# cfpark00/vdm4cdm

Hardware: NVIDIA B200
Metric: denoiser voxel-steps/s at 128^3 (reverse ancestral sampling) (higher is better)
Workload: dtype bf16

## Files before the change

vdm4cdm_b200/csrc/conv3d.cu:

```cuda
#include "common.cuh"
#include "ptx.cuh"
#include "tma_host.cuh"

#ifdef VDM_BRINGUP
#define VDM_DBG(p, f) (((p).debug_flags & (f)) != 0)
#else
#define VDM_DBG(p, f) (false)
#endif

namespace vdm {

constexpr int kConvThreads = 512;
constexpr int kEpiThreads = 256;
constexpr int kEpiFirst = 128;
constexpr int kXfThreads = 128;
constexpr int kXfFirst = 384;
constexpr int kRegsWg0 = 64, kRegsEpi = 176, kRegsXf = 88;
constexpr int kXfGroup = 2;
constexpr int kResSlotBytes = 2 * 16 * kEpiThreads;
constexpr int kMaxBStages = 16;
constexpr int kMaxAStages = 4;
constexpr int kTileH = 16, kTileW = 8;

struct ConvKernelParams {
// ... 918 lines not shown
                issue_fold_stage<MT, KJ, NF>(a_st + kh * (uint32_t)(kTileW + 2) + kw, b_base16 + sb * b_stage16 + b_lbo, a_hi32,
                                             b_hi32, d_tmem0, kc == 0 && khw == 0);
                ptx::umma_commit(&sh->b_empty[sb]);
              }
              ptx::umma_commit(&sh->a_empty[sa]);
              if (kc == k_chunks - 1) ptx::umma_commit(&sh->tmem_full[acc]);
            }
            __syncwarp();
          }
        }
      } else {
      Ring ra(nsa_u);
      for (int tile = blockIdx.x; tile < p.n_tiles; tile += gridDim.x, ++ti) {
        const uint32_t acc = ti & 1;
        ptx::mbar_wait(&sh->tmem_empty[acc], ((ti >> 1) & 1) ^ 1);
        if (ti == 0) ptx::mbar_wait(&sh->b_full[0], 0);
        const uint32_t d_tmem0 = tmem_u + acc * (uint32_t)(MT * NF);
        const int total_chunks = k_chunks + p.skip_chunks;
        for (int kc = 0; kc < total_chunks; ++kc, ra.next()) {
          const uint32_t sa = ra.s;
          ptx::mbar_wait(&a_rdy[sa], ra.ph);
          ptx::tc_fence_after();
          if (leader) {
            if (kc == 0)
              issue_fold_tile<MT, KJ, NF, true>(a_base16 + sa * a_stage16, b_base16, a_hi, b_hi, d_tmem0);
            else if (kc < k_chunks)
              issue_fold_tile<MT, KJ, NF, false>(a_base16 + sa * a_stage16, b_base16 + (uint32_t)kc * chunk_b16, a_hi, b_hi,
                                                 d_tmem0);
            else
              issue_skip_chunk<MT, KJ, NF>(a_base16 + sa * a_stage16,
                                           b_base16 + ((uint32_t)p.b_stage_bytes >> 4) + (uint32_t)(kc - k_chunks) * (2u * KJ * NF),
                                           d_tmem0);
            ptx::umma_commit(&sh->a_empty[sa]);
            if (kc == total_chunks - 1) ptx::umma_commit(&sh->tmem_full[acc]);
          }
          __syncwarp();
        }
      }
      }
    } else {
      const bool res = p.b_resident != 0;
      if (!p.pad) {
        if (res) issue_generic_tiles<MT, KJ, 0, 1, true, kKind>(p, sh, a_rdy, a_base16, b_base16, tmem_u, leader);
        else issue_generic_tiles<MT, KJ, 0, 1, false, kKind>(p, sh, a_rdy, a_base16, b_base16, tmem_u, leader);
      } else if (p.taps_per_stage == 3) {
        if (res) issue_generic_tiles<MT, KJ, 1, 3, true, kKind>(p, sh, a_rdy, a_base16, b_base16, tmem_u, leader);
        else issue_generic_tiles<MT, KJ, 1, 3, false, kKind>(p, sh, a_rdy, a_base16, b_base16, tmem_u, leader);
      } else {
        if (res) issue_generic_tiles<MT, KJ, 1, 1, true, kKind>(p, sh, a_rdy, a_base16, b_base16, tmem_u, leader);
        else issue_generic_tiles<MT, KJ, 1, 1, false, kKind>(p, sh, a_rdy, a_base16, b_base16, tmem_u, leader);
      }
    }
  }
  } else if (warp >= 12) {
    ptx::setmaxnreg_dec<kRegsXf>();
    if constexpr (!TF32)
      if (p.in_norm) transform_tiles<MT, KJ>(p, sh, a_smem, reinterpret_cast<float*>(smem + p.xf_coef_off));
  } else {
    ptx::setmaxnreg_inc<kRegsEpi>();
    constexpr int P = TF32 ? kEpiF32Planar : 0;
    if (p.out_fp32) epilogue_tiles<MT, kEpiFp32>(p, sh, smem, stat_part, stat_acc, tmem_base);
    else if (p.residual && p.stats) epilogue_tiles<MT, P | kEpiRes | kEpiStats>(p, sh, smem, stat_part, stat_acc, tmem_base);
    else if (p.residual) epilogue_tiles<MT, P | kEpiRes>(p, sh, smem, stat_part, stat_acc, tmem_base);
    else if (p.stats) epilogue_tiles<MT, P | kEpiStats>(p, sh, smem, stat_part, stat_acc, tmem_base);
    else epilogue_tiles<MT, P>(p, sh, smem, stat_part, stat_acc, tmem_base);
  }

  ptx::tc_fence_before();
  __syncthreads();
  if (warp == 1) {
    ptx::tc_fence_after();
    ptx::tmem_dealloc(tmem_base, (uint32_t)p.tmem_cols);
  }
}

#include "conv3d_march.cuh"

struct ConvOverrides {
  int debug_flags;
  int force_mt, force_kc, force_nsplit;
  int no_resident;
  int no_fold;
  int no_march;
};
#ifdef VDM_BRINGUP
static ConvOverrides g_overrides = {};
#else
constexpr ConvOverrides g_overrides = {};
#endif

enum class ConvSchedule {
  kTile,
  kFoldResident,
  kFoldStreamed,
  kMarch,
};

struct ConvPlan {
  ConvSchedule schedule;
  int pad;
  int mt, kc, n_split, n_cta;
  int n_tiles, grid;
  int nsa, nsb, taps_per_stage;
  int a_stage_bytes, b_stage_bytes, b_resident;
  int res_depth, res_ring_off;
  int xf_coef_off;
  size_t smem_bytes;
  int m_units, m_nseg, m_seglen;
  int debug_flags;
};

static int tap_cell(const VdmConvDesc& d, int t) {
  return (d.tap_offset[t][0] + 1) * 9 + (d.tap_offset[t][1] + 1) * 3 + d.tap_offset[t][2] + 1;
}

static int plan_conv(const VdmConvDesc& d, bool has_residual, bool has_skip, bool has_xf, int skip_c_in, int sms, bool tf32,
                     ConvPlan& pl) {
  const ConvOverrides& ov = g_overrides;
  pl = ConvPlan{};
  pl.debug_flags = ov.debug_flags;
  int pad = 0;
  for (int t = 0; t < d.n_taps; ++t)
    if (d.tap_offset[t][0] != 0 || d.tap_offset[t][1] != 0 || d.tap_offset[t][2] != 0) pad = 1;
  if (has_xf && d.circular) {
    set_error("vdm_conv3d: the fused input transform is not available with circular padding");
    return VDM_E_UNSUPPORTED;
  }
  if (has_skip && (skip_c_in > 64 || d.out_fp32)) {
    set_error("vdm_conv3d: the fused skip conv supports bf16 layers with skip_c_in <= 64 only (got %d)", skip_c_in);
    return VDM_E_UNSUPPORTED;
  }
  const int xf_bytes = has_xf ? ((d.c_in * 8 + 15) & ~15) : 0;
  const int res_slot = tf32 ? 2 * kResSlotBytes : kResSlotBytes;
  const int skip_w_bytes = has_skip ? skip_c_in * d.c_out_pad * 2 : 0;

  bool fold = !tf32 && d.n_taps == 27 && pad == 1 && (d.c_out_pad == 16 || d.c_out_pad == 32 || d.c_out_pad == 64) && d.depth >= 3 &&
              ov.no_fold == 0 && ov.force_mt == 0 && ov.force_nsplit == 0;
  const bool streamed = d.c_out_pad == 64;
  int fold_mt = 0, fold_kc = 0;
  if (fold && streamed) {
    fold = d.c_in % 32 == 0 && d.depth >= 4;
    fold_mt = 4; fold_kc = 32;
  } else if (fold) {
    const int budget = 227 * 1024 - 1024 - (int)sizeof(ConvShared) - (2 * 2 * 8 * d.c_out_pad * 4 + 2 * d.c_out_pad * 8) - 256 -
                       (has_residual ? 2 * res_slot : 0) - xf_bytes;
    const int w_bytes = 27 * d.c_in * d.c_out_pad * 2 + skip_w_bytes;
    for (int m = 4; m >= 2 && !fold_mt; --m)
      for (int c = 32; c >= 16 && !fold_mt; c -= 16) {
        if (d.c_in % c != 0 || (has_skip && skip_c_in % c != 0)) continue;
        const int a_stage = (((c / 8) * (m + 2) * (kTileH + 2) * (kTileW + 2) * 16) + 127) & ~127;
        if (2 * a_stage + w_bytes <= budget) { fold_mt = m; fold_kc = c; }
      }
    fold = fold_mt != 0;
  }
  if (fold) {
    unsigned seen = 0;
    for (int t = 0; t < 27; ++t) seen |= 1u << tap_cell(d, t);
    fold = seen == (1u << 27) - 1u;
  }
  pl.schedule = !fold ? ConvSchedule::kTile : streamed ? ConvSchedule::kFoldStreamed
              : d.c_in == fold_kc && ov.no_march == 0 ? ConvSchedule::kMarch : ConvSchedule::kFoldResident;
  const bool resident_fold = pl.schedule == ConvSchedule::kFoldResident || pl.schedule == ConvSchedule::kMarch;

  const int tiles_w = ceil_div(d.width, kTileW), tiles_h = ceil_div(d.height, kTileH);
  int n_split = 1, mt = fold_mt;
  if (!fold) {
    double best = -1.0;
    for (int ns = 1; ns <= 8; ns *= 2) {
      if (d.c_out_pad % (ns * 16) != 0) break;
      const int ncta = d.c_out_pad / ns;
      if (ns > 1 && ncta < 32) break;
      int mt_max = 256 / ncta;
      if (mt_max > 4) mt_max = 4;
      if (mt_max > d.depth) mt_max = d.depth;
      for (int m = 1; m <= mt_max; ++m) {
        const long long tiles = (long long)tiles_w * tiles_h * ceil_div(d.depth, m) * d.batch * ns;
        const long long waves = (tiles + sms - 1) / sms;
        const double active = (double)(tiles < sms ? tiles : sms);
        const double fetch_cyc = 32.0 + ncta / 4.0;
        const double mma_cyc = (double)d.n_taps * (d.c_in / 16) * m * (ncta / 2.0 > fetch_cyc ? ncta / 2.0 : fetch_cyc);
        const double bytes = (double)(m + 2 * pad) * (kTileH + 2 * pad) * (kTileW + 2 * pad) * d.c_in * 2.0 +
                             (double)d.n_taps * d.c_in * ncta * 2.0;
        double bw = 5500.0 / active;
        if (bw > 64.0) bw = 64.0;
        const double cyc = (mma_cyc > bytes / bw ? mma_cyc : bytes / bw) + 2000.0;
        const double total = (double)waves * cyc;
        if (best < 0.0 || total < best * 0.999) {
          best = total;
          n_split = ns;
          mt = m;
        }
      }
    }
  }
  if (ov.force_nsplit > 0) n_split = ov.force_nsplit;
  VDM_CHECK_ARG(d.c_out_pad % (n_split * 16) == 0, "vdm_conv3d: n_split=%d does not divide c_out_pad=%d", n_split,
                d.c_out_pad);
  const int n_cta = d.c_out_pad / n_split;
  if (ov.force_mt > 0) mt = ov.force_mt;
  VDM_CHECK_ARG(mt >= 1 && 2 * mt * n_cta <= 512, "vdm_conv3d: MT=%d does not fit TMEM with N=%d", mt, n_cta);
  const long long n_tiles = (long long)tiles_w * tiles_h * ceil_div(d.depth, mt) * d.batch * n_split;
  VDM_CHECK_ARG(n_tiles < (1ll << 31), "vdm_conv3d: too many tiles");
  if (has_skip && !resident_fold) {
    set_error("vdm_conv3d: the fused skip conv needs the kd-folded schedule with resident weights "
              "(3x3x3, c_out_pad 16 or 32, weights + skip weights fit shared memory); c_in=%d c_out=%d", d.c_in, d.c_out);
    return VDM_E_UNSUPPORTED;
  }
  pl.pad = pad; pl.mt = mt; pl.n_split = n_split; pl.n_cta = n_cta; pl.n_tiles = (int)n_tiles;
  pl.taps_per_stage = (d.n_taps % 3 == 0) ? 3 : 1;

  if (pl.schedule == ConvSchedule::kMarch) {
    const long long cols = (long long)d.batch * tiles_h * tiles_w;
    int nseg_best = 1;
    double best = -1.0;
    for (int nseg = 1; nseg <= ceil_div(d.depth, 4); ++nseg) {
      const int seglen = ceil_div(d.depth, nseg);
      if (ceil_div(d.depth, seglen) != nseg) continue;
      const long long rounds = (cols * nseg + sms - 1) / sms;
      const double cost = (double)rounds * (seglen + 3);
      if (best < 0.0 || cost < best * 0.999) { best = cost; nseg_best = nseg; }
    }
    const long long units = cols * nseg_best;
    VDM_CHECK_ARG(units < (1ll << 31), "vdm_conv3d: too many units");
    pl.kc = fold_kc;
    pl.m_nseg = nseg_best;
    pl.m_seglen = ceil_div(d.depth, nseg_best);
    pl.m_units = (int)units;
    const int stage_bytes = (fold_kc / 8) * (kTileH + 2) * (kTileW + 2) * 16;
    int off = kMarchStages * stage_bytes + 27 * (fold_kc / 8) * n_cta * 16 + skip_w_bytes + (int)sizeof(MarchShared) +
              2 * kMEpiWarps * n_cta * 4 + 2 * n_cta * 8 + kMarchCaddMax * 4;
    off = (off + 15) & ~15;
    if (has_residual) {
      pl.res_ring_off = off;
      pl.res_depth = kMarchResDepth;
      off += kMarchResDepth * (n_cta / 8) * kMEpiThreads * 16;
    }
    pl.smem_bytes = (size_t)off + 1024;
    VDM_CHECK_ARG(pl.smem_bytes <= 227 * 1024, "vdm_conv3d: marching layer does not fit shared memory");
    pl.grid = pl.m_units < sms ? pl.m_units : sms;
    return VDM_OK;
  }

  const int plane_bytes = (mt + 2 * pad) * (kTileH + 2 * pad) * (kTileW + 2 * pad) * 16;
  const int stat_part_bytes = 2 * 2 * 8 * n_cta * 4 + 2 * n_cta * 8;
  const int smem_total = 227 * 1024 - 1024  - (int)sizeof(ConvShared) - stat_part_bytes - 256 - xf_bytes;
  const int smem_budget = smem_total - (has_residual ? (resident_fold ? 2 : 4) * res_slot : 0);
  if (fold) {
    pl.kc = fold_kc;
    pl.a_stage_bytes = ((fold_kc / 8) * plane_bytes + 127) & ~127;
  }
  if (pl.schedule == ConvSchedule::kFoldStreamed) {
    pl.b_stage_bytes = 3 * fold_kc * n_cta * 2;
    pl.nsb = (smem_budget - 2 * pl.a_stage_bytes) / pl.b_stage_bytes;
    if (pl.nsb > kMaxBStages) pl.nsb = kMaxBStages;
    VDM_CHECK_ARG(pl.nsb >= 2, "vdm_conv3d: folded streamed layer does not fit shared memory");
  } else if (pl.schedule == ConvSchedule::kFoldResident) {
    pl.b_stage_bytes = d.n_taps * d.c_in * n_cta * 2;
    pl.nsb = 1;
    pl.b_resident = 1;
    VDM_CHECK_ARG(2 * pl.a_stage_bytes + pl.b_stage_bytes + skip_w_bytes <= smem_budget,
                  "vdm_conv3d: folded layer does not fit shared memory");
  } else {
    for (int c : {64, 32, 16}) {
      if ((ov.force_kc > 0 && c != ov.force_kc) || d.c_in % c != 0) continue;
      const int a_stage = ((c / 8) * plane_bytes + 127) & ~127;
      const int b_stage = pl.taps_per_stage * c * n_cta * 2;
      const int room = smem_budget - 2 * a_stage;
      if (room < 2 * b_stage) continue;
      const long long all_b = (long long)d.n_taps * d.c_in * n_cta * 2;
      pl.kc = c;
      pl.a_stage_bytes = a_stage;
      pl.b_stage_bytes = b_stage;
      pl.b_resident = (n_split == 1 && all_b <= room && ov.no_resident == 0) ? 1 : 0;
      pl.nsb = pl.b_resident ? (int)((all_b + b_stage - 1) / b_stage) : (room / b_stage > kMaxBStages ? kMaxBStages : room / b_stage);
      break;
    }
    VDM_CHECK_ARG(pl.kc > 0, "vdm_conv3d: no channel-chunk size fits shared memory (c_in=%d, N=%d, MT=%d)", d.c_in, n_cta, mt);
  }
  VDM_CHECK_ARG(plane_bytes <= 0x3FFF * 16, "vdm_conv3d: halo plane too large for the descriptor stride field");

  const int fixed = pl.nsb * pl.b_stage_bytes + skip_w_bytes + (has_residual ? 4 * res_slot : 0);
  pl.nsa = 2;
  while (pl.nsa < kMaxAStages && (pl.nsa + 1) * pl.a_stage_bytes + fixed <= smem_total) ++pl.nsa;
  const int used = pl.nsa * pl.a_stage_bytes + pl.nsb * pl.b_stage_bytes + skip_w_bytes;
  if (has_residual) {
    const int depth = (smem_total - used) / res_slot;
    pl.res_depth = depth > 4 ? 4 : depth;
    VDM_CHECK_ARG(pl.res_depth >= 1, "vdm_conv3d: no shared memory left for the residual ring");
    pl.res_ring_off = (used + (int)sizeof(ConvShared) + stat_part_bytes + 15) & ~15;
  }
  pl.xf_coef_off = (used + (int)sizeof(ConvShared) + stat_part_bytes + 16 + pl.res_depth * res_slot + 15) & ~15;
  pl.smem_bytes = (size_t)pl.xf_coef_off + xf_bytes + 1024;
  pl.grid = pl.n_tiles < sms ? pl.n_tiles : sms;
  return VDM_OK;
}

static int launch_conv(const ConvPlan& pl, const CUtensorMap& tmx, const CUtensorMap& tmx2, const ConvKernelParams& p,
                       bool tf32, cudaStream_t stream) {
  if (pl.schedule == ConvSchedule::kMarch) {
    const bool sk = p.skip_chunks > 0, xf = p.in_norm != nullptr;
#define VDM_MARCH(KJv, NFv, SKv, XFv)                                                                          \
    if (pl.kc == 16 * KJv && pl.n_cta == NFv && sk == SKv && xf == XFv)                                        \
      return launch_kernel<conv3d_march_kernel<KJv, NFv, SKv, XFv>>(pl.grid, kConvThreads, pl.smem_bytes, stream, tmx, tmx2, p);
#define VDM_MARCH4(SKv, XFv) VDM_MARCH(1, 16, SKv, XFv) VDM_MARCH(1, 32, SKv, XFv) VDM_MARCH(2, 16, SKv, XFv) VDM_MARCH(2, 32, SKv, XFv)
    VDM_MARCH4(false, false) VDM_MARCH4(true, false) VDM_MARCH4(false, true) VDM_MARCH4(true, true)
#undef VDM_MARCH4
#undef VDM_MARCH
    set_error("vdm_conv3d: no marching kernel instance for KC=%d N=%d", pl.kc, pl.n_cta);
    return VDM_E_UNSUPPORTED;
  }
  const int nf = pl.schedule == ConvSchedule::kTile ? 0 : pl.n_cta;
  if (tf32) {
#define VDM_TILE_TF32(MTv, KJv)                                                                                \
    if (pl.mt == MTv && pl.kc == 16 * KJv && nf == 0)                                                          \
      return launch_kernel<conv3d_planar_kernel<MTv, KJv, 0, true>>(pl.grid, kConvThreads, pl.smem_bytes, stream, tmx, tmx2, p);
    VDM_TILE_TF32(1, 1) VDM_TILE_TF32(1, 2) VDM_TILE_TF32(1, 4)
    VDM_TILE_TF32(2, 1) VDM_TILE_TF32(2, 2) VDM_TILE_TF32(2, 4)
    VDM_TILE_TF32(3, 1) VDM_TILE_TF32(3, 2) VDM_TILE_TF32(3, 4)
    VDM_TILE_TF32(4, 1) VDM_TILE_TF32(4, 2) VDM_TILE_TF32(4, 4)
#undef VDM_TILE_TF32
    set_error("vdm_conv3d_tf32: no kernel instance for MT=%d KC=%d", pl.mt, pl.kc / 2);
    return VDM_E_UNSUPPORTED;
  }
#define VDM_TILE(MTv, KJv, NFv)                                                                                \
  if (pl.mt == MTv && pl.kc == 16 * KJv && nf == NFv)                                                          \
    return launch_kernel<conv3d_planar_kernel<MTv, KJv, NFv>>(pl.grid, kConvThreads, pl.smem_bytes, stream, tmx, tmx2, p);
  VDM_TILE(1, 1, 0) VDM_TILE(1, 2, 0) VDM_TILE(1, 4, 0)
  VDM_TILE(2, 1, 0) VDM_TILE(2, 2, 0) VDM_TILE(2, 4, 0)
  VDM_TILE(3, 1, 0) VDM_TILE(3, 2, 0) VDM_TILE(3, 4, 0)
  VDM_TILE(4, 1, 0) VDM_TILE(4, 2, 0) VDM_TILE(4, 4, 0)
  VDM_TILE(4, 1, 16) VDM_TILE(4, 1, 32) VDM_TILE(4, 2, 16) VDM_TILE(4, 2, 32) VDM_TILE(4, 2, 64)
  VDM_TILE(3, 1, 16) VDM_TILE(3, 1, 32) VDM_TILE(3, 2, 16) VDM_TILE(3, 2, 32)
  VDM_TILE(2, 1, 16) VDM_TILE(2, 1, 32) VDM_TILE(2, 2, 16) VDM_TILE(2, 2, 32)
#undef VDM_TILE
  set_error("vdm_conv3d: no kernel instance for MT=%d KC=%d", pl.mt, pl.kc);
  return VDM_E_UNSUPPORTED;
}

}

using namespace vdm;

#ifdef VDM_BRINGUP
extern "C" int vdm_debug_set(int key, int value) {
  switch (key) {
    case 0: return VDM_OK;
    case 1: g_overrides.force_mt = value; return VDM_OK;
    case 2: g_overrides.force_kc = value; return VDM_OK;
    case 3: g_overrides.force_nsplit = value; return VDM_OK;
    case 4: g_overrides.no_resident = value; return VDM_OK;
    case 5: g_overrides.debug_flags = value; return VDM_OK;
    case 6: g_overrides.no_fold = value; return VDM_OK;
    case 7: g_overrides.no_march = value; return VDM_OK;
    default: set_error("vdm_debug_set: unknown key %d", key); return VDM_E_BADARG;
  }
}
#endif

static int conv3d_run(const VdmConvDesc& d, const void* x, const void* w, void* y, const VdmConvEpilogue* epi, bool tf32,
                      cudaStream_t stream) {
  VDM_CHECK_ARG(d.batch >= 1 && d.depth >= 1 && d.height >= 1 && d.width >= 1, "vdm_conv3d: bad grid");
  VDM_CHECK_ARG(d.c_in >= 16 && d.c_in % 16 == 0, "vdm_conv3d: c_in=%d must be a multiple of 16", d.c_in);
  VDM_CHECK_ARG(d.c_out_pad >= 16 && d.c_out_pad % 16 == 0 && d.c_out_pad <= 256,
                "vdm_conv3d: c_out_pad=%d must be a multiple of 16 in [16,256]", d.c_out_pad);
  VDM_CHECK_ARG(d.c_out >= 1 && d.c_out <= d.c_out_pad, "vdm_conv3d: c_out=%d vs c_out_pad=%d", d.c_out, d.c_out_pad);
  VDM_CHECK_ARG(d.out_fp32 || d.c_out % 8 == 0, "vdm_conv3d: bf16 planar output needs c_out %% 8 == 0 (got %d)", d.c_out);
  VDM_CHECK_ARG(d.n_taps >= 1 && d.n_taps <= VDM_MAX_TAPS, "vdm_conv3d: n_taps=%d", d.n_taps);
  const int halo = d.circular ? 1 : 0;
  const int x_planes = d.x_planes > 0 ? d.x_planes : d.c_in / 8;
  const int y_planes = d.y_planes > 0 ? d.y_planes : (d.c_out + 7) / 8;
  VDM_CHECK_ARG(d.x_plane0 >= 0 && d.x_plane0 + d.c_in / 8 <= x_planes, "vdm_conv3d: x plane window out of range");
  VDM_CHECK_ARG(d.out_fp32 || (d.y_plane0 >= 0 && d.y_plane0 + d.c_out / 8 <= y_planes),
                "vdm_conv3d: y plane window out of range");
  VDM_CHECK_ARG((reinterpret_cast<uintptr_t>(x) & 15) == 0 && (reinterpret_cast<uintptr_t>(w) & 15) == 0 &&
                    (reinterpret_cast<uintptr_t>(y) & 15) == 0,
                "vdm_conv3d: pointers must be 16-byte aligned");
  VDM_CHECK_ARG((long long)d.batch * x_planes < (1ll << 31), "vdm_conv3d: too many planes");
  for (int t = 0; t < d.n_taps; ++t)
    for (int k = 0; k < 3; ++k)
      VDM_CHECK_ARG(d.tap_offset[t][k] >= -1 && d.tap_offset[t][k] <= 1, "vdm_conv3d: tap offset out of range");
  const bool has_residual = epi && epi->residual;
  const bool has_skip = epi && epi->skip_x;
  const bool has_xf = epi && epi->in_norm;
  VDM_CHECK_ARG(!has_skip || (epi->skip_w && epi->skip_c_in >= 16 && epi->skip_c_in % 16 == 0),
                "vdm_conv3d: fused skip conv needs packed weights and skip_c_in a multiple of 16, got %d", epi->skip_c_in);
  if (!encode_fn()) {
    set_error("vdm_conv3d: cuTensorMapEncodeTiled is not available from the driver");
    return VDM_E_DRIVER;
  }

  ConvPlan pl;
  const int rc = plan_conv(d, has_residual, has_skip, has_xf, has_skip ? epi->skip_c_in : 0, num_sms(), tf32, pl);
  if (rc != VDM_OK) return rc;
  const int x2_planes = !has_skip ? 0 : epi->skip_planes > 0 ? epi->skip_planes : epi->skip_c_in / 8;
  VDM_CHECK_ARG(!has_skip || (epi->skip_plane0 >= 0 && epi->skip_plane0 + epi->skip_c_in / 8 <= x2_planes),
                "vdm_conv3d: skip plane window out of range");
  VDM_CHECK_ARG(!(epi && epi->stats && d.out_fp32), "vdm_conv3d: stats are only produced for bf16 outputs");
  VDM_CHECK_ARG(!(has_residual && d.out_fp32), "vdm_conv3d: residual is only supported for bf16 outputs");
  VDM_CHECK_ARG(!(has_residual && epi->residual_upsample) || (d.depth % 2 == 0 && d.height % 2 == 0 && d.width % 2 == 0),
                "vdm_conv3d: an up-sampled residual needs an even grid, got (%d,%d,%d)", d.depth, d.height, d.width);
  const bool march = pl.schedule == ConvSchedule::kMarch;

  ConvKernelParams p;
  memset(&p, 0, sizeof(p));
  p.B = d.batch; p.D = d.depth; p.H = d.height; p.W = d.width;
  p.c_out = d.c_out; p.n_pad = d.c_out_pad; p.n_taps = d.n_taps; p.pad = pl.pad;
  p.n_split = pl.n_split; p.n_cta = pl.n_cta;
  p.MT = pl.mt; p.KC = pl.kc; p.k_chunks = d.c_in / pl.kc;
  p.tiles_w = ceil_div(d.width, kTileW); p.tiles_h = ceil_div(d.height, kTileH); p.tiles_d = ceil_div(d.depth, pl.mt);
  p.n_tiles = pl.n_tiles;
  p.fast_div_ok = pl.n_tiles < (1 << 22) ? 1 : 0;
  p.inv_n_split = 1.0f / (float)pl.n_split; p.inv_tiles_w = 1.0f / (float)p.tiles_w;
  p.inv_tiles_h = 1.0f / (float)p.tiles_h; p.inv_tiles_d = 1.0f / (float)p.tiles_d;
  p.Hd = pl.mt + 2 * pl.pad; p.Hh = kTileH + 2 * pl.pad; p.Wh = kTileW + 2 * pl.pad;
  p.plane_bytes = p.Hd * p.Hh * p.Wh * 16;
  for (int t = 0; t < d.n_taps; ++t)
    p.tap16[t] = (uint16_t)(((d.tap_offset[t][0] + pl.pad) * p.Hh + (d.tap_offset[t][1] + pl.pad)) * p.Wh + d.tap_offset[t][2] + pl.pad);
  if (pl.schedule != ConvSchedule::kTile)
    for (int t = 0; t < 27; ++t) {
      const int c = tap_cell(d, t);
      p.tap_kd[t] = (int8_t)(c / 9);
      p.tap_khw[t] = (int8_t)(c % 9);
      p.tap_of[c / 9][c % 9] = (int8_t)t;
    }
  p.fold_streamed = pl.schedule == ConvSchedule::kFoldStreamed ? 1 : 0;
  p.nsa = pl.nsa; p.nsb = pl.nsb; p.taps_per_stage = pl.taps_per_stage;
  p.a_stage_bytes = pl.a_stage_bytes; p.b_stage_bytes = pl.b_stage_bytes; p.b_resident = pl.b_resident;
  int cols = 32;
  while (cols < 2 * pl.mt * pl.n_cta) cols <<= 1;
  p.tmem_cols = cols;
  p.c_in = d.c_in; p.c_in8 = d.c_in / 8;
  p.x_planes = x_planes; p.x_plane0 = d.x_plane0;
  p.x_shift = halo;
  if (has_skip) {
    p.skip_chunks = epi->skip_c_in / pl.kc;
    p.skip_w_bytes = epi->skip_c_in * d.c_out_pad * 2;
    p.w2 = static_cast<const __nv_bfloat16*>(epi->skip_w);
    p.x2_planes = x2_planes;
    p.x2_plane0 = epi->skip_plane0;
  }
  p.w = static_cast<const __nv_bfloat16*>(w);
  p.y = y; p.y_planes = y_planes; p.y_plane0 = d.y_plane0; p.out_fp32 = d.out_fp32;
  if (epi) {
    p.chan_add = epi->chan_add;
    p.step_ptr = epi->step_ptr;
    p.chan_add_step_stride = epi->chan_add_step_stride;
    p.residual = static_cast<const __nv_bfloat16*>(epi->residual);
    p.r_planes = d.r_planes > 0 ? d.r_planes : d.c_out / 8;
    p.r_plane0 = d.r_plane0;
    p.r_up = (epi->residual && epi->residual_upsample) ? 1 : 0;
    p.r_d2s_planes = (epi->residual && epi->residual_upsample == 2) ? d.c_out / 8 : 0;
    p.stats = epi->stats;
    p.stats_channels = epi->stats_channels > 0 ? epi->stats_channels : d.c_out;
    p.stats_c0 = epi->stats_c0;
    p.in_norm = epi->in_norm;
  }
  p.res_depth = pl.res_depth; p.res_ring_off = pl.res_ring_off; p.xf_coef_off = pl.xf_coef_off;
  p.m_units = pl.m_units; p.m_nseg = pl.m_nseg; p.m_seglen = pl.m_seglen;
  p.debug_flags = pl.debug_flags;

  const uint32_t box_d = march ? 1u : (uint32_t)p.Hd, planes = (uint32_t)(pl.kc / 8);
  CUtensorMap tmx, tmx2;
  int e = encode_planar(&tmx, x, d.width + 2 * halo, d.height + 2 * halo, d.depth + 2 * halo, (uint64_t)d.batch * x_planes,
                        0, {(uint32_t)p.Wh, (uint32_t)p.Hh, box_d, planes}, "vdm_conv3d", march ? "x, marching" : "x");
  if (e != VDM_OK) return e;
  tmx2 = tmx;
  if (has_skip) {
    e = encode_planar(&tmx2, epi->skip_x, d.width, d.height, d.depth, (uint64_t)d.batch * x2_planes, 0,
                      {(uint32_t)kTileW, (uint32_t)kTileH, march ? 1u : (uint32_t)pl.mt, planes}, "vdm_conv3d",
                      march ? "skip_x, marching" : "skip_x");
    if (e != VDM_OK) return e;
  }
  return launch_conv(pl, tmx, tmx2, p, tf32, stream);
}

extern "C" int vdm_conv3d(const VdmConvDesc* desc, const void* x, const void* w, void* y,
                          const VdmConvEpilogue* epi, void* stream) {
  VDM_CHECK_ARG(desc && x && w && y, "vdm_conv3d: NULL pointer argument");
  return conv3d_run(*desc, x, w, y, epi, false, (cudaStream_t)stream);
}

extern "C" int vdm_conv3d_tf32(const VdmConvDesc* desc, const void* x, const void* w, void* y,
                               const VdmConvEpilogue* epi, void* stream) {
  VDM_CHECK_ARG(desc && x && w && y, "vdm_conv3d_tf32: NULL pointer argument");
// ... 16 lines not shown
```

vdm4cdm_b200/csrc/conv3d_march.cuh:

```cuda
#pragma once

constexpr int kMarchStages = 8;
constexpr int kMarchBlocks = 16;
constexpr int kMEpiWarps = 12, kMEpiThreads = 384;
constexpr int kRegsMEpi = 144;
constexpr int kMarchResDepth = 2;
constexpr int kMarchCaddMax = 1024;

struct MarchShared {
  uint64_t a_full[kMarchStages], a_empty[kMarchStages];
  uint64_t a_ready[kMarchStages];
  uint64_t b_full;
  uint64_t t_full[kMarchBlocks], t_empty[kMarchBlocks];
  uint32_t tmem_base;
};

struct MarchUnit {
  int b, h0, w0, d0, len;
};
__device__ __forceinline__ MarchUnit decode_unit(const ConvKernelParams& p, int u) {
  MarchUnit m;
  const int seg = u % p.m_nseg; u /= p.m_nseg;
  m.w0 = (u % p.tiles_w) * kTileW; u /= p.tiles_w;
  m.h0 = (u % p.tiles_h) * kTileH;
// ... 235 lines not shown
          stat_acc[c] = a1;
          stat_acc[NF + c] = a2;
        }
      }
      asm volatile("bar.sync 2, %0;" ::"n"(kThreadsE) : "memory");
    }
  }
}

template <int KJ, bool SKIP, int NXW>
__device__ __forceinline__ void march_transform(const ConvKernelParams& p, MarchShared* sh, uint8_t* a_smem) {
  constexpr int planes = 2 * KJ, S = kMarchStages;
  constexpr int kSliceBytes = (kTileH + 2) * (kTileW + 2) * 16, kStageBytes = planes * kSliceBytes;
  constexpr int lpp = 32 / planes;
  constexpr int nvox = (kTileH + 2) * (kTileW + 2);
  constexpr int KMAX0 = (nvox + lpp - 1) / lpp;
  constexpr int G = planes == 2 ? 6 : 8;
  constexpr int KMAX = (KMAX0 + G - 1) / G * G;
  static_assert(KMAX <= 32, "one bit per voxel of a lane in zmask");
  const int lane = threadIdx.x & 31, j = (threadIdx.x >> 5) - (16 - NXW);
  const int pl = lane / lpp, l0 = lane % lpp;
  const int skip_chunks = SKIP ? p.skip_chunks : 0;
  float ca[8], cb[8];
  int cur_b = -1;
  uint32_t it = 0, n_main = 0, n_skip = 0;
  for (int u = blockIdx.x; u < p.m_units; u += gridDim.x) {
    const MarchUnit m = decode_unit(p, u);
    if (m.b != cur_b) {
      cur_b = m.b;
      const float4* cs = reinterpret_cast<const float4*>(p.in_norm + ((long long)m.b * p.c_in + pl * 8) * 2);
#pragma unroll
      for (int j4 = 0; j4 < 4; ++j4) {
        const float4 c4 = __ldg(cs + j4);
        ca[2 * j4] = c4.x; cb[2 * j4] = c4.y; ca[2 * j4 + 1] = c4.z; cb[2 * j4 + 1] = c4.w;
      }
    }
    uint32_t zmask = 0u;
    if (m.h0 == 0 || m.h0 + kTileH >= p.H || m.w0 == 0 || m.w0 + kTileW >= p.W) {
      for (int k = 0; k < KMAX; ++k) {
        const int v = l0 + k * lpp;
        const int hy = v / (kTileW + 2), wx = v - hy * (kTileW + 2);
        if (v < nvox && ((unsigned)(m.h0 - 1 + hy) >= (unsigned)p.H || (unsigned)(m.w0 - 1 + wx) >= (unsigned)p.W)) zmask |= 1u << k;
      }
    }
    for (int i = 0; i < m.len + 2; ++i, ++n_main) {
      if ((int)(n_main % (uint32_t)NXW) == j) {
        const uint32_t s = it % (uint32_t)S;
        ptx::mbar_wait(&sh->a_full[s], (it / (uint32_t)S) & 1);
        const int dz = m.d0 - 1 + i;
        if (dz >= 0 && dz < p.D) {
          uint4* base = reinterpret_cast<uint4*>(a_smem + (size_t)s * kStageBytes + (size_t)pl * kSliceBytes);
#pragma unroll 1
          for (int k0 = 0; k0 < KMAX; k0 += G) {
            uint4 xs[G];
#pragma unroll
            for (int g2 = 0; g2 < G; ++g2) xs[g2] = base[l0 + (k0 + g2) * lpp];
#pragma unroll
            for (int g2 = 0; g2 < G; ++g2) {
              const int v = l0 + (k0 + g2) * lpp;
              uint4 y = gn_silu8(xs[g2], ca, cb);
              if ((zmask >> (k0 + g2)) & 1u) y = make_uint4(0u, 0u, 0u, 0u);
              if (v < nvox) base[v] = y;
            }
          }
        }
        ptx::fence_proxy_async();
        __syncwarp();
        if (lane == 0) ptx::mbar_arrive(&sh->a_ready[s]);
      }
      ++it;
      if (i < m.len) {
        for (int c = 0; c < skip_chunks; ++c, ++it, ++n_skip) {
          if ((int)(n_skip % (uint32_t)NXW) == j) {
            const uint32_t s = it % (uint32_t)S;
            ptx::mbar_wait(&sh->a_full[s], (it / (uint32_t)S) & 1);
            if (lane == 0) ptx::mbar_arrive(&sh->a_ready[s]);
          }
        }
      }
    }
  }
}

template <int KJ, int NF, bool SKIP, bool XF>
__global__ void __launch_bounds__(kConvThreads, 1)
conv3d_march_kernel(const __grid_constant__ CUtensorMap tmap_x, const __grid_constant__ CUtensorMap tmap_x2,
                    const __grid_constant__ ConvKernelParams p) {
  extern __shared__ __align__(1024) uint8_t smem_raw[];
  uint8_t* smem = smem_raw + ((1024u - (ptx::smem_u32(smem_raw) & 1023u)) & 1023u);
  constexpr int planes = 2 * KJ;
  constexpr int kSliceBytes = (kTileH + 2) * (kTileW + 2) * 16;
  constexpr int kStageBytes = planes * kSliceBytes;
  constexpr int kWBytes = 27 * planes * NF * 16;
  constexpr int R = kMarchBlocks, S = kMarchStages;
  uint8_t* a_smem = smem;
  uint8_t* b_smem = smem + (size_t)S * kStageBytes;
  MarchShared* sh = reinterpret_cast<MarchShared*>(b_smem + kWBytes + p.skip_w_bytes);
  float* stat_part = reinterpret_cast<float*>(sh + 1);
  double* stat_acc = reinterpret_cast<double*>(stat_part + 2 * kMEpiWarps * NF);
  float* cadd_s = reinterpret_cast<float*>(stat_acc + 2 * NF);

  const int warp = threadIdx.x >> 5;
  const int lane = threadIdx.x & 31;
  if (threadIdx.x == 0) {
    ptx::prefetch_tensormap(&tmap_x);
    for (int s = 0; s < S; ++s) {
      ptx::mbar_init(&sh->a_full[s], 1);
      ptx::mbar_init(&sh->a_empty[s], 1);
      ptx::mbar_init(&sh->a_ready[s], 1);
    }
    ptx::mbar_init(&sh->b_full, 1);
    for (int g = 0; g < R; ++g) {
      ptx::mbar_init(&sh->t_full[g], 1);
      ptx::mbar_init(&sh->t_empty[g], 128);
    }
    ptx::fence_barrier_init();
  }
  if (warp == 1) {
    ptx::tmem_alloc(&sh->tmem_base, (uint32_t)(R * NF));
    ptx::tmem_relinquish();
  }
  if (warp >= 4) {
    for (int i = threadIdx.x - kEpiFirst; i < 2 * NF; i += kMEpiThreads) stat_acc[i] = 0.0;
  }
  ptx::tc_fence_before();
  __syncthreads();
  ptx::tc_fence_after();
  const uint32_t tmem_base = sh->tmem_base;

  if (warp < 4) {
    ptx::setmaxnreg_dec<kRegsWg0>();
    if (warp == 0) {
      if (lane == 0) {
        uint32_t it = 0;
        for (int u = blockIdx.x; u < p.m_units; u += gridDim.x) {
          const MarchUnit m = decode_unit(p, u);
          for (int i = 0; i < m.len + 2; ++i) {
            {
              const int s = (int)(it % (uint32_t)S);
              ptx::mbar_wait(&sh->a_empty[s], ((it / (uint32_t)S) & 1) ^ 1);
              if (VDM_DBG(p, 2) && it >= (uint32_t)S) {
                ptx::mbar_arrive(&sh->a_full[s]);
              } else {
                ptx::mbar_arrive_expect_tx(&sh->a_full[s], (uint32_t)kStageBytes);
                ptx::tma_load_4d(a_smem + (size_t)s * kStageBytes, &tmap_x, &sh->a_full[s], (m.w0 - 1 + p.x_shift) * 8,
                                 m.h0 - 1 + p.x_shift, m.d0 - 1 + i + p.x_shift, m.b * p.x_planes + p.x_plane0);
              }
              ++it;
            }
            if (i < m.len) {
              for (int c = 0; c < (SKIP ? p.skip_chunks : 0); ++c, ++it) {
                const int s = (int)(it % (uint32_t)S);
                ptx::mbar_wait(&sh->a_empty[s], ((it / (uint32_t)S) & 1) ^ 1);
                ptx::mbar_arrive_expect_tx(&sh->a_full[s], (uint32_t)(planes * kTileH * kTileW * 16));
                ptx::tma_load_4d(a_smem + (size_t)s * kStageBytes, &tmap_x2, &sh->a_full[s], m.w0 * 8, m.h0, m.d0 + i,
                                 m.b * p.x2_planes + p.x2_plane0 + c * planes);
              }
            }
          }
        }
      }
    } else if (warp == 2) {
      if (lane == 0 && blockIdx.x < (unsigned)p.m_units) {
        const size_t tap_stride = (size_t)p.c_in8 * p.n_pad * 8, plane_stride = (size_t)p.n_pad * 8;
        ptx::mbar_arrive_expect_tx(&sh->b_full, (uint32_t)kWBytes + (uint32_t)p.skip_w_bytes);
        for (int pl = 0; pl < p.skip_chunks * planes; ++pl)
          ptx::bulk_load(b_smem + kWBytes + (size_t)pl * (NF * 16), p.w2 + (size_t)pl * plane_stride, (uint32_t)(NF * 16), &sh->b_full);
        for (int tap = 0; tap < 27; ++tap) {
          const int kd = p.tap_kd[tap], khw = p.tap_khw[tap];
#pragma unroll
          for (int pl = 0; pl < planes; ++pl)
            ptx::bulk_load(b_smem + (size_t)((khw * planes + pl) * 3 + (2 - kd)) * (NF * 16),
                           p.w + (size_t)tap * tap_stride + (size_t)pl * plane_stride, (uint32_t)(NF * 16), &sh->b_full);
        }
      }
    } else if (warp == 1) {
      const uint32_t a_base16 = ptx::smem_u32(a_smem) >> 4, a_stage16 = (uint32_t)kStageBytes >> 4;
      const uint32_t b_base16 = ptx::smem_u32(b_smem) >> 4;
      const uint32_t tmem_u = __shfl_sync(0xffffffffu, tmem_base, 0);
      const bool leader = ptx::elect_one();
      const uint64_t a_hi = make_planar_desc(0, (uint32_t)kSliceBytes, (uint32_t)(kTileW + 2) * 16u);
      const uint64_t b_hi = make_planar_desc(0, 3u * (uint32_t)NF * 16u, 128u);
      const uint64_t b_desc0 = b_hi | (uint64_t)b_base16;
      if (leader && blockIdx.x < (unsigned)p.m_units) {
        ptx::mbar_wait(&sh->b_full, 0);
        int u = blockIdx.x;
        MarchUnit m = decode_unit(p, u);
        const int skip_chunks = SKIP ? p.skip_chunks : 0;
        uint32_t ita = 0, ob = 0;
        auto wait_stage = [&](uint32_t ita_) __attribute__((always_inline)) {
          ptx::mbar_wait(XF ? &sh->a_ready[ita_ % (uint32_t)S] : &sh->a_full[ita_ % (uint32_t)S], (ita_ / (uint32_t)S) & 1);
          ptx::tc_fence_after();
        };
        auto wait_skip_stage = [&](uint32_t ita_) __attribute__((always_inline)) { wait_stage(ita_); };
        auto wait_block = [&](uint32_t o) __attribute__((always_inline)) {
          ptx::mbar_wait(&sh->t_empty[o % (uint32_t)R], ((o / (uint32_t)R) & 1) ^ 1);
        };
        auto wait_slice = [&](int ii, uint32_t ita_, uint32_t ob_, int len_) __attribute__((always_inline)) {
          if (ii < len_) wait_block(ob_ + (uint32_t)ii);
          wait_stage(ita_);
        };
        const uint64_t a2_hi = make_planar_desc(0, (uint32_t)(kTileH * kTileW * 16), (uint32_t)kTileW * 16u);
        const uint64_t b2_hi = make_planar_desc(0, (uint32_t)NF * 16u, 128u);
        const uint32_t b2_base16 = b_base16 + ((uint32_t)kWBytes >> 4);
        auto skip_stages = [&](int i, int len) __attribute__((always_inline)) {
          const uint32_t d_s = tmem_u + ((ob + (uint32_t)i) % (uint32_t)R) * (uint32_t)NF;
          for (int c = 0; c < skip_chunks; ++c, ++ita) {
            const uint32_t s2 = ita % (uint32_t)S;
            const uint64_t a2 = a2_hi | (uint64_t)(a_base16 + s2 * a_stage16);
            const uint64_t b2 = b2_hi | (uint64_t)(b2_base16 + (uint32_t)(c * planes * NF));
#pragma unroll
            for (int j = 0; j < KJ; ++j)
              ptx::umma_bf16_off64(d_s, 0u, a2, (uint32_t)(j * 2 * kTileH * kTileW), b2, (uint32_t)(2 * j * NF),
                                   ptx::make_idesc_bf16(128, (uint32_t)NF), 1u);
            if (c + 1 < skip_chunks) wait_skip_stage(ita + 1u);
            else wait_slice(i + 1, ita + 1u, ob, len);
            ptx::umma_commit(&sh->a_empty[s2]);
          }
        };
        wait_slice(0, 0u, 0u, m.len);
        while (true) {
          const int len = m.len;
          const int nu = u + (int)gridDim.x;
          const bool more_units = nu < p.m_units;
          MarchUnit nm = m;
          if (more_units) nm = decode_unit(p, nu);
          auto general_slice = [&](int i) __attribute__((always_inline)) {
            const uint32_t sa = ita % (uint32_t)S;
            const uint64_t a_desc = a_hi | (uint64_t)(a_base16 + sa * a_stage16);
            const bool last = i == len + 1;
            const bool skip_next = SKIP && i < len;
            const int s_lo = i - 2 > 0 ? i - 2 : 0, s_hi = i < len - 1 ? i : len - 1;
            const bool fresh = i < len;
            const uint32_t g_lo = (ob + (uint32_t)s_lo) % (uint32_t)R;
            const int n = s_hi - s_lo + 1;
            const int n1 = n < R - (int)g_lo ? n : R - (int)g_lo;
            const uint64_t b_desc = b_desc0 + (uint64_t)((2 - i + s_lo) * NF);
            issue_march_slice<KJ, NF, 0, 5>(a_desc, b_desc, tmem_u, g_lo, n, n1, fresh);
            if (skip_next) wait_skip_stage(ita + 1u);
            else if (!last) wait_slice(i + 1, ita + 1u, ob, len);
            else if (more_units) wait_slice(0, ita + 1u, ob + (uint32_t)len, nm.len);
            issue_march_slice<KJ, NF, 5, 9>(a_desc, b_desc, tmem_u, g_lo, n, n1, fresh);
            ptx::umma_commit(&sh->a_empty[sa]);
            if (i >= 2) ptx::umma_commit(&sh->t_full[(ob + (uint32_t)(i - 2)) % (uint32_t)R]);
            ++ita;
            if (skip_next) skip_stages(i, len);
          };
          int i = 0;
          for (; i < 2 && i < len + 2; ++i) general_slice(i);
          for (; i < len; ++i) {
            const uint32_t g_st = (ob + (uint32_t)(i - 2)) % (uint32_t)R;
            if (g_st > (uint32_t)(R - 3)) {
              general_slice(i);
              continue;
            }
            const uint32_t sa = ita % (uint32_t)S;
            const uint64_t a_desc = a_hi | (uint64_t)(a_base16 + sa * a_stage16);
            const uint32_t d_col = tmem_u + g_st * (uint32_t)NF;
            issue_march_span<KJ, NF, true, 0, 2, 3>(a_desc, b_desc0, d_col, 3);
            if (!SKIP && i + 1 < len) wait_block(ob + (uint32_t)(i + 1));
            issue_march_span<KJ, NF, true, 2, 4, 3>(a_desc, b_desc0, d_col, 3);
            if (SKIP) wait_skip_stage(ita + 1u);
            else wait_stage(ita + 1u);
            issue_march_span<KJ, NF, true, 4, 6, 3>(a_desc, b_desc0, d_col, 3);
            issue_march_span<KJ, NF, true, 6, 9, 3>(a_desc, b_desc0, d_col, 3);
            ptx::umma_commit(&sh->a_empty[sa]);
            ptx::umma_commit(&sh->t_full[g_st]);
            ++ita;
            if (SKIP) skip_stages(i, len);
          }
          for (; i < len + 2; ++i) general_slice(i);
          if (!more_units) break;
          ob += (uint32_t)len;
          u = nu;
          m = nm;
        }
      }
      __syncwarp();
    }
  } else {
    ptx::setmaxnreg_inc<kRegsMEpi>();
    constexpr bool kWideXf = XF && !SKIP && NF == 16;
    if (kWideXf && p.out_fp32) {
      if (warp >= 8) march_transform<KJ, SKIP, 8>(p, sh, a_smem);
      else march_epilogue<NF, kEpiFp32, 1>(p, sh, smem, stat_part, stat_acc, cadd_s, tmem_base);
    } else if (XF && warp >= 12) {
      march_transform<KJ, SKIP, 4>(p, sh, a_smem);
    } else {
      constexpr int EW = XF ? 2 : 3;
      if (p.out_fp32) march_epilogue<NF, kEpiFp32, EW>(p, sh, smem, stat_part, stat_acc, cadd_s, tmem_base);
      else if (p.residual && p.stats) march_epilogue<NF, kEpiRes | kEpiStats, EW>(p, sh, smem, stat_part, stat_acc, cadd_s, tmem_base);
      else if (p.residual) march_epilogue<NF, kEpiRes, EW>(p, sh, smem, stat_part, stat_acc, cadd_s, tmem_base);
      else if (p.stats) march_epilogue<NF, kEpiStats, EW>(p, sh, smem, stat_part, stat_acc, cadd_s, tmem_base);
      else march_epilogue<NF, 0, EW>(p, sh, smem, stat_part, stat_acc, cadd_s, tmem_base);
    }
  }

  ptx::tc_fence_before();
  __syncthreads();
  if (warp == 1) {
    ptx::tc_fence_after();
    ptx::tmem_dealloc(tmem_base, (uint32_t)(R * NF));
  }
}
```

Before: 1.581 billion.

## Add tap-stacked marching conv kernel for single-channel fp32 output layer

```diff
diff --git a/vdm4cdm_b200/csrc/conv3d.cu b/vdm4cdm_b200/csrc/conv3d.cu
--- a/vdm4cdm_b200/csrc/conv3d.cu
+++ b/vdm4cdm_b200/csrc/conv3d.cu
@@ -1024,6 +1024,7 @@
   int no_resident;
   int no_fold;
   int no_march;
+  int no_march_taps;
 };
 #ifdef VDM_BRINGUP
 static ConvOverrides g_overrides = {};
@@ -1036,6 +1037,7 @@
   kFoldResident,
   kFoldStreamed,
   kMarch,
+  kMarchTaps,
 };
 
 struct ConvPlan {
@@ -1102,7 +1104,10 @@
   }
   pl.schedule = !fold ? ConvSchedule::kTile : streamed ? ConvSchedule::kFoldStreamed
               : d.c_in == fold_kc && ov.no_march == 0 ? ConvSchedule::kMarch : ConvSchedule::kFoldResident;
-  const bool resident_fold = pl.schedule == ConvSchedule::kFoldResident || pl.schedule == ConvSchedule::kMarch;
+  if (pl.schedule == ConvSchedule::kMarch && d.c_out == 1 && d.c_out_pad == 16 && d.out_fp32 && ov.no_march_taps == 0)
+    pl.schedule = ConvSchedule::kMarchTaps;
+  const bool march = pl.schedule == ConvSchedule::kMarch || pl.schedule == ConvSchedule::kMarchTaps;
+  const bool resident_fold = pl.schedule == ConvSchedule::kFoldResident || march;
 
   const int tiles_w = ceil_div(d.width, kTileW), tiles_h = ceil_div(d.height, kTileH);
   int n_split = 1, mt = fold_mt;
@@ -1151,7 +1156,7 @@
   pl.pad = pad; pl.mt = mt; pl.n_split = n_split; pl.n_cta = n_cta; pl.n_tiles = (int)n_tiles;
   pl.taps_per_stage = (d.n_taps % 3 == 0) ? 3 : 1;
 
-  if (pl.schedule == ConvSchedule::kMarch) {
+  if (march) {
     const long long cols = (long long)d.batch * tiles_h * tiles_w;
     int nseg_best = 1;
     double best = -1.0;
@@ -1169,6 +1174,11 @@
     pl.m_seglen = ceil_div(d.depth, nseg_best);
     pl.m_units = (int)units;
     const int stage_bytes = (fold_kc / 8) * (kTileH + 2) * (kTileW + 2) * 16;
+    if (pl.schedule == ConvSchedule::kMarchTaps) {
+      pl.smem_bytes = (size_t)(kMarchStages * stage_bytes + (fold_kc / 8) * 32 * 16 + 2 * kTapsPBytes) + sizeof(MarchShared) + 1024;
+      pl.grid = pl.m_units < sms ? pl.m_units : sms;
+      return VDM_OK;
+    }
     int off = kMarchStages * stage_bytes + 27 * (fold_kc / 8) * n_cta * 16 + skip_w_bytes + (int)sizeof(MarchShared) +
               2 * kMEpiWarps * n_cta * 4 + 2 * n_cta * 8 + kMarchCaddMax * 4;
     off = (off + 15) & ~15;
@@ -1251,6 +1261,16 @@
     set_error("vdm_conv3d: no marching kernel instance for KC=%d N=%d", pl.kc, pl.n_cta);
     return VDM_E_UNSUPPORTED;
   }
+  if (pl.schedule == ConvSchedule::kMarchTaps) {
+    const bool xf = p.in_norm != nullptr;
+#define VDM_MARCH_TAPS(KJv, XFv)                                                                               \
+    if (pl.kc == 16 * KJv && xf == XFv)                                                                        \
+      return launch_kernel<conv3d_march_taps_kernel<KJv, XFv>>(pl.grid, kConvThreads, pl.smem_bytes, stream, tmx, tmx2, p);
+    VDM_MARCH_TAPS(1, false) VDM_MARCH_TAPS(2, false) VDM_MARCH_TAPS(1, true) VDM_MARCH_TAPS(2, true)
+#undef VDM_MARCH_TAPS
+    set_error("vdm_conv3d: no tap-stacked marching kernel instance for KC=%d", pl.kc);
+    return VDM_E_UNSUPPORTED;
+  }
   const int nf = pl.schedule == ConvSchedule::kTile ? 0 : pl.n_cta;
   if (tf32) {
 #define VDM_TILE_TF32(MTv, KJv)                                                                                \
@@ -1294,6 +1314,7 @@
     case 5: g_overrides.debug_flags = value; return VDM_OK;
     case 6: g_overrides.no_fold = value; return VDM_OK;
     case 7: g_overrides.no_march = value; return VDM_OK;
+    case 8: g_overrides.no_march_taps = value; return VDM_OK;
     default: set_error("vdm_debug_set: unknown key %d", key); return VDM_E_BADARG;
   }
 }
@@ -1341,7 +1362,7 @@
   VDM_CHECK_ARG(!(has_residual && d.out_fp32), "vdm_conv3d: residual is only supported for bf16 outputs");
   VDM_CHECK_ARG(!(has_residual && epi->residual_upsample) || (d.depth % 2 == 0 && d.height % 2 == 0 && d.width % 2 == 0),
                 "vdm_conv3d: an up-sampled residual needs an even grid, got (%d,%d,%d)", d.depth, d.height, d.width);
-  const bool march = pl.schedule == ConvSchedule::kMarch;
+  const bool march = pl.schedule == ConvSchedule::kMarch || pl.schedule == ConvSchedule::kMarchTaps;
 
   ConvKernelParams p;
   memset(&p, 0, sizeof(p));
diff --git a/vdm4cdm_b200/csrc/conv3d_march.cuh b/vdm4cdm_b200/csrc/conv3d_march.cuh
--- a/vdm4cdm_b200/csrc/conv3d_march.cuh
+++ b/vdm4cdm_b200/csrc/conv3d_march.cuh
@@ -341,6 +341,40 @@
   }
 }
 
+template <int KJ, bool SKIP>
+__device__ __forceinline__ void march_produce_a(const ConvKernelParams& p, MarchShared* sh, uint8_t* a_smem,
+                                                const CUtensorMap* tmap_x, const CUtensorMap* tmap_x2) {
+  constexpr int planes = 2 * KJ, S = kMarchStages;
+  constexpr int kStageBytes = planes * (kTileH + 2) * (kTileW + 2) * 16;
+  uint32_t it = 0;
+  for (int u = blockIdx.x; u < p.m_units; u += gridDim.x) {
+    const MarchUnit m = decode_unit(p, u);
+    for (int i = 0; i < m.len + 2; ++i) {
+      {
+        const int s = (int)(it % (uint32_t)S);
+        ptx::mbar_wait(&sh->a_empty[s], ((it / (uint32_t)S) & 1) ^ 1);
+        if (VDM_DBG(p, 2) && it >= (uint32_t)S) {
+          ptx::mbar_arrive(&sh->a_full[s]);
+        } else {
+          ptx::mbar_arrive_expect_tx(&sh->a_full[s], (uint32_t)kStageBytes);
+          ptx::tma_load_4d(a_smem + (size_t)s * kStageBytes, tmap_x, &sh->a_full[s], (m.w0 - 1 + p.x_shift) * 8,
+                           m.h0 - 1 + p.x_shift, m.d0 - 1 + i + p.x_shift, m.b * p.x_planes + p.x_plane0);
+        }
+        ++it;
+      }
+      if (i < m.len) {
+        for (int c = 0; c < (SKIP ? p.skip_chunks : 0); ++c, ++it) {
+          const int s = (int)(it % (uint32_t)S);
+          ptx::mbar_wait(&sh->a_empty[s], ((it / (uint32_t)S) & 1) ^ 1);
+          ptx::mbar_arrive_expect_tx(&sh->a_full[s], (uint32_t)(planes * kTileH * kTileW * 16));
+          ptx::tma_load_4d(a_smem + (size_t)s * kStageBytes, tmap_x2, &sh->a_full[s], m.w0 * 8, m.h0, m.d0 + i,
+                           m.b * p.x2_planes + p.x2_plane0 + c * planes);
+        }
+      }
+    }
+  }
+}
+
 template <int KJ, int NF, bool SKIP, bool XF>
 __global__ void __launch_bounds__(kConvThreads, 1)
 conv3d_march_kernel(const __grid_constant__ CUtensorMap tmap_x, const __grid_constant__ CUtensorMap tmap_x2,
@@ -390,35 +424,7 @@
   if (warp < 4) {
     ptx::setmaxnreg_dec<kRegsWg0>();
     if (warp == 0) {
-      if (lane == 0) {
-        uint32_t it = 0;
-        for (int u = blockIdx.x; u < p.m_units; u += gridDim.x) {
-          const MarchUnit m = decode_unit(p, u);
-          for (int i = 0; i < m.len + 2; ++i) {
-            {
-              const int s = (int)(it % (uint32_t)S);
-              ptx::mbar_wait(&sh->a_empty[s], ((it / (uint32_t)S) & 1) ^ 1);
-              if (VDM_DBG(p, 2) && it >= (uint32_t)S) {
-                ptx::mbar_arrive(&sh->a_full[s]);
-              } else {
-                ptx::mbar_arrive_expect_tx(&sh->a_full[s], (uint32_t)kStageBytes);
-                ptx::tma_load_4d(a_smem + (size_t)s * kStageBytes, &tmap_x, &sh->a_full[s], (m.w0 - 1 + p.x_shift) * 8,
-                                 m.h0 - 1 + p.x_shift, m.d0 - 1 + i + p.x_shift, m.b * p.x_planes + p.x_plane0);
-              }
-              ++it;
-            }
-            if (i < m.len) {
-              for (int c = 0; c < (SKIP ? p.skip_chunks : 0); ++c, ++it) {
-                const int s = (int)(it % (uint32_t)S);
-                ptx::mbar_wait(&sh->a_empty[s], ((it / (uint32_t)S) & 1) ^ 1);
-                ptx::mbar_arrive_expect_tx(&sh->a_full[s], (uint32_t)(planes * kTileH * kTileW * 16));
-                ptx::tma_load_4d(a_smem + (size_t)s * kStageBytes, &tmap_x2, &sh->a_full[s], m.w0 * 8, m.h0, m.d0 + i,
-                                 m.b * p.x2_planes + p.x2_plane0 + c * planes);
-              }
-            }
-          }
-        }
-      }
+      if (lane == 0) march_produce_a<KJ, SKIP>(p, sh, a_smem, &tmap_x, &tmap_x2);
     } else if (warp == 2) {
       if (lane == 0 && blockIdx.x < (unsigned)p.m_units) {
         const size_t tap_stride = (size_t)p.c_in8 * p.n_pad * 8, plane_stride = (size_t)p.n_pad * 8;
@@ -562,3 +568,178 @@
     ptx::tmem_dealloc(tmem_base, (uint32_t)(R * NF));
   }
 }
+
+constexpr int kTapsRing = 4;
+constexpr int kTapsVox = (kTileH + 2) * (kTileW + 2);
+constexpr int kTapsPBytes = 27 * kTapsVox * 4;
+
+__device__ __forceinline__ void march_taps_epilogue(const ConvKernelParams& p, MarchShared* sh, float* pbuf,
+                                                    const uint32_t tmem_base) {
+  const int warp = threadIdx.x >> 5, lane = threadIdx.x & 31;
+  const int q = warp & 3;
+  const int v0 = q * 32 + lane, v1 = 128 + q * 32 + lane;
+  const int oh = q + 4 * (lane >> 3), ow = lane & 7;
+  const int vo = oh * (kTileW + 2) + ow;
+  const long long HW = (long long)p.H * p.W, V = (long long)p.D * HW;
+  const long long cadd_step = (p.chan_add && p.step_ptr) ? (long long)(*p.step_ptr) : 0ll;
+  const float* cadd_g = p.chan_add ? p.chan_add + cadd_step * p.chan_add_step_stride : nullptr;
+  const uint32_t trow = tmem_base + ((uint32_t)(q * 32) << 16);
+  uint32_t it = 0;
+  for (int u = blockIdx.x; u < p.m_units; u += gridDim.x) {
+    const MarchUnit m = decode_unit(p, u);
+    const int h = m.h0 + oh, w = m.w0 + ow;
+    const bool hw_ok = (h < p.H) && (w < p.W);
+    const float bias = cadd_g ? __ldg(cadd_g + m.b) : 0.f;
+    float* y = static_cast<float*>(p.y) + (long long)m.b * V + ((long long)m.d0 * p.H + h) * p.W + w;
+    float acc1 = 0.f, acc0 = 0.f;
+    for (int i = 0; i < m.len + 2; ++i, ++it) {
+      const uint32_t g = it % (uint32_t)kTapsRing;
+      ptx::mbar_wait(&sh->t_full[g], (it / (uint32_t)kTapsRing) & 1);
+      ptx::tc_fence_after();
+      const uint32_t tcol = trow + g * 64u;
+      uint32_t r0[16], r1[16], r2[16], r3[16];
+      ptx::tmem_ld16(tcol, r0);
+      ptx::tmem_ld16(tcol + 16u, r1);
+      if (q < 2) {
+        ptx::tmem_ld16(tcol + 32u, r2);
+        ptx::tmem_ld16(tcol + 48u, r3);
+      }
+      ptx::tmem_ld_wait_dep(r0);
+      ptx::tmem_ld_wait_dep(r1);
+      if (q < 2) {
+        ptx::tmem_ld_wait_dep(r2);
+        ptx::tmem_ld_wait_dep(r3);
+      }
+      ptx::tc_fence_before();
+      ptx::mbar_arrive(&sh->t_empty[g]);
+      float* P = pbuf + (it & 1u) * (27 * kTapsVox);
+#pragma unroll
+      for (int t = 0; t < 27; ++t) P[t * kTapsVox + v0] = __uint_as_float(t < 16 ? r0[t] : r1[t - 16]);
+      if (q < 2 && v1 < kTapsVox) {
+#pragma unroll
+        for (int t = 0; t < 27; ++t) P[t * kTapsVox + v1] = __uint_as_float(t < 16 ? r2[t] : r3[t - 16]);
+      }
+      asm volatile("bar.sync 1, 128;" ::: "memory");
+      float qk[3];
+#pragma unroll
+      for (int kd = 0; kd < 3; ++kd) {
+        float s = 0.f;
+#pragma unroll
+        for (int khw = 0; khw < 9; ++khw)
+          s += P[(kd * 9 + khw) * kTapsVox + vo + (khw / 3) * (kTileW + 2) + khw % 3];
+        qk[kd] = s;
+      }
+      const float out = acc1 + qk[2];
+      acc1 = acc0 + qk[1];
+      acc0 = qk[0];
+      if (i >= 2 && hw_ok) y[(long long)(i - 2) * HW] = out + bias;
+    }
+  }
+}
+
+template <int KJ, bool XF>
+__global__ void __launch_bounds__(kConvThreads, 1)
+conv3d_march_taps_kernel(const __grid_constant__ CUtensorMap tmap_x, const __grid_constant__ CUtensorMap tmap_x2,
+                         const __grid_constant__ ConvKernelParams p) {
+  extern __shared__ __align__(1024) uint8_t smem_raw[];
+  uint8_t* smem = smem_raw + ((1024u - (ptx::smem_u32(smem_raw) & 1023u)) & 1023u);
+  constexpr int planes = 2 * KJ, S = kMarchStages;
+  constexpr int kSliceBytes = kTapsVox * 16;
+  constexpr int kStageBytes = planes * kSliceBytes;
+  constexpr int kWBytes = planes * 32 * 16;
+  constexpr uint32_t kTmemCols = kTapsRing * 64;
+  uint8_t* a_smem = smem;
+  uint8_t* b_smem = smem + (size_t)S * kStageBytes;
+  float* pbuf = reinterpret_cast<float*>(b_smem + kWBytes);
+  MarchShared* sh = reinterpret_cast<MarchShared*>(b_smem + kWBytes + 2 * kTapsPBytes);
+
+  const int warp = threadIdx.x >> 5;
+  const int lane = threadIdx.x & 31;
+  if (threadIdx.x == 0) {
+    ptx::prefetch_tensormap(&tmap_x);
+    for (int s = 0; s < S; ++s) {
+      ptx::mbar_init(&sh->a_full[s], 1);
+      ptx::mbar_init(&sh->a_empty[s], 1);
+      ptx::mbar_init(&sh->a_ready[s], 1);
+    }
+    ptx::mbar_init(&sh->b_full, 1);
+    for (int g = 0; g < kTapsRing; ++g) {
+      ptx::mbar_init(&sh->t_full[g], 1);
+      ptx::mbar_init(&sh->t_empty[g], 128);
+    }
+    ptx::fence_barrier_init();
+  }
+  if (warp == 1) {
+    ptx::tmem_alloc(&sh->tmem_base, kTmemCols);
+    ptx::tmem_relinquish();
+  }
+  if (warp == 3 && lane < planes * 5) {
+    const int pl = lane / 5, col = 27 + lane % 5;
+    *reinterpret_cast<uint4*>(b_smem + (pl * 32 + col) * 16) = make_uint4(0u, 0u, 0u, 0u);
+    ptx::fence_proxy_async();
+  }
+  ptx::tc_fence_before();
+  __syncthreads();
+  ptx::tc_fence_after();
+  const uint32_t tmem_base = sh->tmem_base;
+
+  if (warp < 4) {
+    ptx::setmaxnreg_dec<kRegsWg0>();
+    if (warp == 0) {
+      if (lane == 0) march_produce_a<KJ, false>(p, sh, a_smem, &tmap_x, &tmap_x2);
+    } else if (warp == 2) {
+      if (lane == 0 && blockIdx.x < (unsigned)p.m_units) {
+        const size_t tap_stride = (size_t)p.c_in8 * p.n_pad * 8, plane_stride = (size_t)p.n_pad * 8;
+        ptx::mbar_arrive_expect_tx(&sh->b_full, (uint32_t)(27 * planes * 16));
+        for (int tap = 0; tap < 27; ++tap) {
+          const int col = p.tap_kd[tap] * 9 + p.tap_khw[tap];
+#pragma unroll
+          for (int pl = 0; pl < planes; ++pl)
+            ptx::bulk_load(b_smem + (size_t)(pl * 32 + col) * 16, p.w + (size_t)tap * tap_stride + (size_t)pl * plane_stride, 16u,
+                           &sh->b_full);
+        }
+      }
+    } else if (warp == 1) {
+      const uint32_t a_base16 = ptx::smem_u32(a_smem) >> 4, a_stage16 = (uint32_t)kStageBytes >> 4;
+      const uint64_t a_hi = make_planar_desc(0, (uint32_t)kSliceBytes, 128u);
+      const uint64_t b_desc = make_planar_desc(0, 32u * 16u, 128u) | (uint64_t)(ptx::smem_u32(b_smem) >> 4);
+      const uint32_t idesc = ptx::make_idesc_bf16(128, 32);
+      const uint32_t tmem_u = __shfl_sync(0xffffffffu, tmem_base, 0);
+      const bool leader = ptx::elect_one();
+      if (leader && blockIdx.x < (unsigned)p.m_units) {
+        ptx::mbar_wait(&sh->b_full, 0);
+        uint32_t it = 0;
+        for (int u = blockIdx.x; u < p.m_units; u += gridDim.x) {
+          const int n = decode_unit(p, u).len + 2;
+          for (int i = 0; i < n; ++i, ++it) {
+            const uint32_t sa = it % (uint32_t)S, g = it % (uint32_t)kTapsRing;
+            ptx::mbar_wait(XF ? &sh->a_ready[sa] : &sh->a_full[sa], (it / (uint32_t)S) & 1);
+            ptx::mbar_wait(&sh->t_empty[g], ((it / (uint32_t)kTapsRing) & 1) ^ 1);
+            ptx::tc_fence_after();
+            const uint64_t a_desc = a_hi | (uint64_t)(a_base16 + sa * a_stage16);
+#pragma unroll
+            for (int mb = 0; mb < 2; ++mb)
+#pragma unroll
+              for (int j = 0; j < KJ; ++j)
+                ptx::umma_bf16_off64(tmem_u + g * 64u, (uint32_t)(mb * 32), a_desc, (uint32_t)(mb * 128 + j * 2 * kTapsVox),
+                                     b_desc, (uint32_t)(j * 64), idesc, j > 0 ? 1u : 0u);
+            ptx::umma_commit(&sh->a_empty[sa]);
+            ptx::umma_commit(&sh->t_full[g]);
+          }
+        }
+      }
+      __syncwarp();
+    }
+  } else {
+    ptx::setmaxnreg_inc<kRegsMEpi>();
+    if (warp < 8) march_taps_epilogue(p, sh, pbuf, tmem_base);
+    else if (XF) march_transform<KJ, false, 8>(p, sh, a_smem);
+  }
+
+  ptx::tc_fence_before();
+  __syncthreads();
+  if (warp == 1) {
+    ptx::tc_fence_after();
+    ptx::tmem_dealloc(tmem_base, kTmemCols);
+  }
+}
```

Measured after the change: 1.585 billion (median of 6 runs). Within noise of the previous version (+0.3%).
